# alibaba/unified-audio

Hardware: NVIDIA H100
Metric: hcodec2_encode_rvq_decode_samples_per_s (higher is better)
Workload: dtype f16x3/f16 tensor-core, f32 accumulate

## Files before the change

### unified_audio_b200/csrc/common.cuh

```cuda
#pragma once
#include <cuda.h>
#include <cuda_fp16.h>
#include <cuda_runtime.h>
#include <stdint.h>

namespace qb {

void set_error(const char* fmt, ...);
#define QB_CHECK_CUDA(expr)                                                              \
  do {                                                                                   \
    cudaError_t _e = (expr);                                                             \
    if (_e != cudaSuccess) {                                                             \
      qb::set_error("%s:%d CUDA error %s: %s", __FILE__, __LINE__, #expr, cudaGetErrorString(_e)); \
      return -2;                                                                         \
    }                                                                                    \
  } while (0)
#define QB_REQUIRE(cond, ...)                                                            \
  do {                                                                                   \
    if (!(cond)) {                                                                       \
      qb::set_error(__VA_ARGS__);                                                        \
      return -1;                                                                         \
    }                                                                                    \
  } while (0)

static inline int64_t ceil_div(int64_t a, int64_t b) { return (a + b - 1) / b; }

__device__ __forceinline__ float gelu_erf(float x) { return 0.5f * x * (1.0f + erff(x * 0.70710678118654752440f)); }
__device__ __forceinline__ float gelu_fast(float x) {
  const float z = fabsf(x) * 0.70710678118654752440f;
  float t;
  asm("rcp.approx.ftz.f32 %0, %1;" : "=f"(t) : "f"(fmaf(0.3275911f, z, 1.0f)));
  float p = fmaf(1.061405429f, t, -1.453152027f);
  p = fmaf(p, t, 1.421413741f);
  p = fmaf(p, t, -0.284496736f);
  p = fmaf(p, t, 0.254829592f);
  p *= t;
  float e;
  asm("ex2.approx.ftz.f32 %0, %1;" : "=f"(e) : "f"(-1.4426950408889634f * z * z));
  const float erf_abs = fmaf(-p, e, 1.0f);
  const float half_x = 0.5f * x;
  return fmaf(fabsf(half_x), erf_abs, half_x);
}
__device__ __forceinline__ float sigmoid_f(float x) { return 1.0f / (1.0f + __expf(-x)); }
__device__ __forceinline__ float sigmoid_acc(float x) { return 1.0f / (1.0f + expf(-x)); }
#ifndef LM_ATT_U_DEFAULT
#define LM_ATT_U_DEFAULT 8
#endif
__device__ __forceinline__ float silu_f(float x) { return x / (1.0f + expf(-x)); }
__device__ __forceinline__ float elu_f(float x) { return x > 0.f ? x : expm1f(x); }

__device__ __forceinline__ __half f2h_sat(float x) {
  unsigned short h;
  asm("cvt.rn.satfinite.f16.f32 %0, %1;" : "=h"(h) : "f"(x));
  return __ushort_as_half(h);
}
__device__ __forceinline__ void split_f16(float x, __half& hi, __half& lo) {
  hi = f2h_sat(x);
  lo = __float2half_rn(x - __half2float(hi));
}

__device__ __forceinline__ float warp_sum(float v) {
#pragma unroll
  for (int o = 16; o > 0; o >>= 1) v += __shfl_xor_sync(0xffffffffu, v, o);
  return v;
}
__device__ __forceinline__ float warp_max(float v) {
#pragma unroll
  for (int o = 16; o > 0; o >>= 1) v = fmaxf(v, __shfl_xor_sync(0xffffffffu, v, o));
  return v;
}

__device__ __forceinline__ uint32_t smem_u32(const void* p) { return (uint32_t)__cvta_generic_to_shared(p); }

__device__ __forceinline__ bool elect_one() {
  uint32_t pred;
  asm volatile(
      "{\n\t.reg .pred P;\n\t elect.sync _|P, 0xffffffff;\n\t selp.u32 %0, 1, 0, P;\n\t}\n"
      : "=r"(pred));
  return pred != 0;
}

__device__ __forceinline__ void mbar_init(uint64_t* bar, uint32_t count) {
  asm volatile("mbarrier.init.shared::cta.b64 [%0], %1;" ::"r"(smem_u32(bar)), "r"(count));
}
__device__ __forceinline__ void fence_mbar_init() { asm volatile("fence.mbarrier_init.release.cluster;" ::: "memory"); }
__device__ __forceinline__ void fence_proxy_async() { asm volatile("fence.proxy.async.shared::cta;" ::: "memory"); }
__device__ __forceinline__ void mbar_arrive_expect_tx(uint64_t* bar, uint32_t bytes) {
  asm volatile("mbarrier.arrive.expect_tx.shared::cta.b64 _, [%0], %1;" ::"r"(smem_u32(bar)), "r"(bytes) : "memory");
}
__device__ __forceinline__ void mbar_arrive(uint64_t* bar) {
  asm volatile("mbarrier.arrive.shared::cta.b64 _, [%0];" ::"r"(smem_u32(bar)) : "memory");
}
__device__ __forceinline__ bool mbar_try_wait(uint64_t* bar, uint32_t parity) {
  uint32_t ok;
  asm volatile(
      "{\n\t.reg .pred P;\n\t"
      "mbarrier.try_wait.parity.shared::cta.b64 P, [%1], %2;\n\t"
      "selp.u32 %0, 1, 0, P;\n\t}\n"
      : "=r"(ok)
      : "r"(smem_u32(bar)), "r"(parity)
      : "memory");
  return ok != 0;
}
__device__ __forceinline__ void mbar_wait(uint64_t* bar, uint32_t parity) {
  uint32_t spins = 0;
  while (!mbar_try_wait(bar, parity)) {
    if (++spins > (1u << 26)) { asm volatile("trap;"); }
  }
}

__device__ __forceinline__ void mbar_wait_parked(uint64_t* bar, uint32_t parity) {
  uint32_t spins = 0;
  for (;;) {
    uint32_t ok;
    asm volatile(
        "{\n\t.reg .pred P;\n\t"
        "mbarrier.try_wait.parity.shared::cta.b64 P, [%1], %2, %3;\n\t"
        "selp.u32 %0, 1, 0, P;\n\t}\n"
        : "=r"(ok)
        : "r"(smem_u32(bar)), "r"(parity), "r"(200000u)
        : "memory");
    if (ok) return;
    if (++spins > (1u << 22)) { asm volatile("trap;"); }
  }
}

template <int N>
__device__ __forceinline__ void setmaxnreg_inc() { asm volatile("setmaxnreg.inc.sync.aligned.u32 %0;" ::"n"(N)); }
template <int N>
__device__ __forceinline__ void setmaxnreg_dec() { asm volatile("setmaxnreg.dec.sync.aligned.u32 %0;" ::"n"(N)); }

__device__ __forceinline__ void prefetch_tmap(const void* tmap) {
  asm volatile("prefetch.tensormap [%0];" ::"l"(tmap) : "memory");
}
__device__ __forceinline__ void tma_load_2d(void* smem_dst, const void* tmap, uint64_t* bar, int x, int y) {
  asm volatile(
      "cp.async.bulk.tensor.2d.shared::cluster.global.mbarrier::complete_tx::bytes [%0], [%1, {%3, %4}], [%2];"
      ::"r"(smem_u32(smem_dst)), "l"(tmap), "r"(smem_u32(bar)), "r"(x), "r"(y)
      : "memory");
}
__device__ __forceinline__ void tma_load_3d(void* smem_dst, const void* tmap, uint64_t* bar, int x, int y, int z) {
  asm volatile(
      "cp.async.bulk.tensor.3d.shared::cluster.global.mbarrier::complete_tx::bytes [%0], [%1, {%3, %4, %5}], [%2];"
      ::"r"(smem_u32(smem_dst)), "l"(tmap), "r"(smem_u32(bar)), "r"(x), "r"(y), "r"(z)
      : "memory");
}
__device__ __forceinline__ void tma_store_3d(const void* tmap, const void* smem_src, int x, int y, int z) {
  asm volatile("cp.async.bulk.tensor.3d.global.shared::cta.bulk_group [%0, {%2, %3, %4}], [%1];"
               ::"l"(tmap), "r"(smem_u32(smem_src)), "r"(x), "r"(y), "r"(z)
               : "memory");
}
__device__ __forceinline__ void bulk_commit() { asm volatile("cp.async.bulk.commit_group;" ::: "memory"); }
template <int N>
__device__ __forceinline__ void bulk_wait_read() { asm volatile("cp.async.bulk.wait_group.read %0;" ::"n"(N) : "memory"); }
template <int N>
__device__ __forceinline__ void bulk_wait() { asm volatile("cp.async.bulk.wait_group %0;" ::"n"(N) : "memory"); }
__device__ __forceinline__ void st_shared_f32x2(uint32_t addr, float x, float y) {
  asm volatile("st.shared.v2.f32 [%0], {%1, %2};" ::"r"(addr), "f"(x), "f"(y));
}
__device__ __forceinline__ float2 ld_shared_f32x2(uint32_t addr) {
  float2 v;
  asm volatile("ld.shared.v2.f32 {%0, %1}, [%2];" : "=f"(v.x), "=f"(v.y) : "r"(addr));
  return v;
}
__device__ __forceinline__ void st_shared_b32(uint32_t addr, uint32_t v) {
  asm volatile("st.shared.b32 [%0], %1;" ::"r"(addr), "r"(v));
}
__device__ __forceinline__ void named_bar_sync(int id, int count) {
  asm volatile("bar.sync %0, %1;" ::"r"(id), "r"(count) : "memory");
}

}
```

### unified_audio_b200/csrc/gemm.cu

```cuda
#include <cstdarg>
#include <cstdio>
#include <cstdlib>
#include <cstring>
#include <atomic>

#include "common.cuh"
#include "quark_b200.h"
#include "wgmma.cuh"

namespace qb {

static thread_local char g_err[1024] = "";
std::atomic<long long> g_launches{0};
void set_error(const char* fmt, ...) {
  va_list ap;
  va_start(ap, fmt);
  vsnprintf(g_err, sizeof(g_err), fmt, ap);
  va_end(ap);
}

constexpr int QB_MAX_DEVICES = 64;
static int current_device() {
  int dev = 0;
  cudaGetDevice(&dev);
  return dev >= 0 && dev < QB_MAX_DEVICES ? dev : 0;
}

#ifndef QB_PARK
#define QB_PARK 1
#endif

enum EpiKind : int { EPI_GENERIC = 0, EPI_HI = 1, EPI_F32 = 2 };

struct RowMapD {
  void* ptr;
  long long ld, rpb, off;
};
struct GemmParams {
  int tiles_per_batch, num_n_tiles, num_tiles, num_kb;
  int taps, stride, cblocks, C, dil;
  int Cld;
  int m_per_batch, N;
  const float* bias;
  const float* gamma;
  const float* act_p;
  const float* act2_p;
  RowMapD res, o32, ohi, olo;
  int act, act2;
  int epi;
  const __half *a_hi, *a_lo, *w_hi, *w_lo;
  long long a_rpb;
  int a_batch;
};

__device__ __forceinline__ float snake_f(float v, float a) {
  const float t = a * v;
  float sn;
  if (fabsf(t) < 64.f) {
    const float k = rintf(t * 0.15915494309189535f);
    const float r = fmaf(k, -6.2831854820251465f, t);
    sn = __sinf(fmaf(k, 1.7484555e-7f, r));
  } else {
    sn = sinf(t);
  }
  float rc;
  asm("rcp.approx.ftz.f32 %0, %1;" : "=f"(rc) : "f"(a + 1e-9f));
  return fmaf(rc, sn * sn, v);
}
__device__ __forceinline__ float apply_act(int act, float v) {
  if (act == QB_ACT_GELU) return gelu_fast(v);
  if (act == QB_ACT_ELU) return elu_f(v);
  if (act == QB_ACT_TANH) return tanhf(v);
  if (act == QB_ACT_RELU) return v < 0.f ? 0.f : v;
  return v;
}

__device__ __forceinline__ void epi_finish_scalar(const GemmParams& p, int b, int m, int n, float v) {
  if (p.gamma) v *= __ldg(p.gamma + n);
  if (p.res.ptr) v += ((const float*)p.res.ptr)[((long long)b * p.res.rpb + p.res.off + m) * p.res.ld + n];
  if (p.o32.ptr) ((float*)p.o32.ptr)[((long long)b * p.o32.rpb + p.o32.off + m) * p.o32.ld + n] = v;
  if (p.ohi.ptr) {
    float u = p.act2 == QB_ACT_ELU ? elu_f(v) : (p.act2 == QB_ACT_SNAKE ? snake_f(v, __ldg(p.act2_p + n)) : v);
    __half h, l;
    split_f16(u, h, l);
    long long o = ((long long)b * p.ohi.rpb + p.ohi.off + m) * p.ohi.ld + n;
    ((__half*)p.ohi.ptr)[o] = h;
    if (p.olo.ptr) ((__half*)p.olo.ptr)[o] = l;
  }
}

__device__ __forceinline__ uint8_t* align1024(uint8_t* p) {
  return (uint8_t*)(((uintptr_t)p + 1023) & ~(uintptr_t)1023);
}

__device__ __forceinline__ void epilogue_pair(const GemmParams& p, int b, int m, int n, float v0, float v1) {
  if (m >= p.m_per_batch || n >= p.N) return;
  const bool has1 = n + 1 < p.N;
  if (p.bias) {
    v0 += __ldg(p.bias + n);
    if (has1) v1 += __ldg(p.bias + n + 1);
  }
  if (p.act == QB_ACT_SWIGLU) {
    epi_finish_scalar(p, b, m, n >> 1, silu_f(v0) * v1);
    return;
  }
  if (has1 && p.act2 == QB_ACT_NONE && (p.act == QB_ACT_NONE || p.act == QB_ACT_GELU)) {
    if (p.ohi.ptr && !p.olo.ptr && !p.o32.ptr && !p.res.ptr && !p.gamma && (p.ohi.ld & 1) == 0 &&
        (reinterpret_cast<uintptr_t>(p.ohi.ptr) & 3) == 0) {
      if (p.act == QB_ACT_GELU) { v0 = gelu_fast(v0); v1 = gelu_fast(v1); }
      const __half2 hmax = __float2half2_rn(65504.f), hmin = __float2half2_rn(-65504.f);
      *reinterpret_cast<__half2*>((__half*)p.ohi.ptr + ((long long)b * p.ohi.rpb + p.ohi.off + m) * p.ohi.ld + n) =
          __hmax2_nan(__hmin2_nan(__floats2half2_rn(v0, v1), hmax), hmin);
      return;
    }
    if (p.o32.ptr && !p.ohi.ptr && p.act == QB_ACT_NONE && (p.o32.ld & 1) == 0 && (reinterpret_cast<uintptr_t>(p.o32.ptr) & 7) == 0 &&
        (!p.res.ptr || ((p.res.ld & 1) == 0 && (reinterpret_cast<uintptr_t>(p.res.ptr) & 7) == 0)) &&
        (!p.gamma || (reinterpret_cast<uintptr_t>(p.gamma) & 7) == 0)) {
      if (p.gamma) {
        const float2 g = __ldg(reinterpret_cast<const float2*>(p.gamma + n));
        v0 *= g.x; v1 *= g.y;
      }
      if (p.res.ptr) {
        const float2 r = *reinterpret_cast<const float2*>((const float*)p.res.ptr + ((long long)b * p.res.rpb + p.res.off + m) * p.res.ld + n);
        v0 += r.x; v1 += r.y;
      }
      *reinterpret_cast<float2*>((float*)p.o32.ptr + ((long long)b * p.o32.rpb + p.o32.off + m) * p.o32.ld + n) = make_float2(v0, v1);
      return;
    }
  }
  if (p.act == QB_ACT_SNAKE) {
    v0 = snake_f(v0, __ldg(p.act_p + n));
    if (has1) v1 = snake_f(v1, __ldg(p.act_p + n + 1));
  } else if (p.act != QB_ACT_NONE) {
    v0 = apply_act(p.act, v0);
    v1 = apply_act(p.act, v1);
  }
  epi_finish_scalar(p, b, m, n, v0);
  if (has1) epi_finish_scalar(p, b, m, n + 1, v1);
}

constexpr int GEMM_BM = 128, GEMM_BK = 64;
constexpr int GEMM_THREADS = 3 * 128;
constexpr int GEMM_PRODUCER_REGS = 40, GEMM_CONSUMER_REGS = 232;

constexpr int EPI_BUFS = 2;
constexpr uint32_t EPI_SUB_BYTES = 64 * 128;

template <int BN>
__device__ __forceinline__ void load_tile_cols(const GemmParams& p, int n0, int ct, float (&v)[2 * BN / 256]) {
#pragma unroll
  for (int i = 0; i < 2 * BN / 256; ++i) {
    const int k = ct + 256 * i, n = n0 + k % BN;
    const float* src = k < BN ? p.bias : p.gamma;
    v[i] = src && n < p.N ? __ldg(src + n) : 0.f;
  }
}

struct EpiCtx {
  uint8_t* buf;
  uint64_t* rfull;
  uint32_t cols;
  int cw, b, row0, n0;
};

template <int BN>
__device__ __forceinline__ void epilogue_hi(const GemmParams& p, const CUtensorMap* tmO, const EpiCtx& e, const float (&acc)[BN / 2]) {
  constexpr int NSUB = BN / 64;
  const __half2 hmax = __float2half2_rn(65504.f), hmin = __float2half2_rn(-65504.f);
  const bool gelu = p.act == QB_ACT_GELU, leader = (threadIdx.x & 127) == 0;
  const int lane = threadIdx.x & 31;
  const uint32_t th = smem_u32(e.buf) + (((threadIdx.x >> 5) & 3) * 16 + (lane >> 2)) * 128 + 4 * (lane & 3), sw = (lane >> 2) << 4;
#pragma unroll
  for (int s = 0; s < NSUB; ++s) {
    uint8_t* buf = e.buf + (s % EPI_BUFS) * EPI_SUB_BYTES;
    if (s == 0) {
      if (leader) bulk_wait_read<0>();
      named_bar_sync(2 + e.cw, 128);
    } else if (s >= EPI_BUFS) {
      if (leader) bulk_wait_read<EPI_BUFS - 1>();
      named_bar_sync(2 + e.cw, 128);
    }
#pragma unroll
    for (int jj = 0; jj < 8; ++jj) {
      const int j = 8 * s + jj;
      const float2 bb = p.bias ? ld_shared_f32x2(e.cols + 4 * (8 * j + 2 * (lane & 3))) : make_float2(0.f, 0.f);
#pragma unroll
      for (int h = 0; h < 2; ++h) {
        float v0 = acc[4 * j + 2 * h], v1 = acc[4 * j + 2 * h + 1];
        if (p.bias) { v0 += bb.x; v1 += bb.y; }
        if (gelu) { v0 = gelu_fast(v0); v1 = gelu_fast(v1); }
        const __half2 o = __hmax2_nan(__hmin2_nan(__floats2half2_rn(v0, v1), hmax), hmin);
        st_shared_b32(th + (s % EPI_BUFS) * EPI_SUB_BYTES + h * 1024 + ((16 * jj) ^ sw), *reinterpret_cast<const uint32_t*>(&o));
      }
    }
    fence_proxy_async();
    named_bar_sync(2 + e.cw, 128);
    if (leader) {
      tma_store_3d(tmO, buf, e.n0 + 64 * s, e.row0, e.b);
      bulk_commit();
    }
  }
}

template <int BN>
__device__ __forceinline__ void epilogue_f32(const GemmParams& p, const CUtensorMap* tmO, const CUtensorMap* tmR, const EpiCtx& e,
                                             const float (&acc)[BN / 2]) {
  constexpr int NSUB = BN / 32;
  static_assert(NSUB % (2 * EPI_BUFS) == 0, "each residual barrier completes an even number of phases per tile");
  const bool res = p.res.ptr != nullptr, leader = (threadIdx.x & 127) == 0;
  const int lane = threadIdx.x & 31;
  const uint32_t th = smem_u32(e.buf) + (((threadIdx.x >> 5) & 3) * 16 + (lane >> 2)) * 128 + 8 * (lane & 1),
                 sw = (((lane >> 1) & 1) ^ (lane >> 2)) << 4;
#pragma unroll
  for (int s = 0; s < NSUB; ++s) {
    const int u = s % EPI_BUFS;
    uint8_t* buf = e.buf + u * EPI_SUB_BYTES;
    if (res) {
      mbar_wait(&e.rfull[u], (s / EPI_BUFS) & 1);
    } else if (s == 0) {
      if (leader) bulk_wait_read<0>();
      named_bar_sync(2 + e.cw, 128);
    } else if (s >= EPI_BUFS) {
      if (leader) bulk_wait_read<EPI_BUFS - 1>();
      named_bar_sync(2 + e.cw, 128);
    }
#pragma unroll
    for (int jj = 0; jj < 4; ++jj) {
      const int j = 4 * s + jj;
      const uint32_t col = e.cols + 4 * (8 * j + 2 * (lane & 3));
      const float2 bb = p.bias ? ld_shared_f32x2(col) : make_float2(0.f, 0.f);
      const float2 g = p.gamma ? ld_shared_f32x2(col + 4 * BN) : make_float2(1.f, 1.f);
#pragma unroll
      for (int h = 0; h < 2; ++h) {
        const uint32_t el = th + u * EPI_SUB_BYTES + h * 1024 + ((32 * jj) ^ sw);
        float v0 = acc[4 * j + 2 * h], v1 = acc[4 * j + 2 * h + 1];
        if (p.bias) { v0 += bb.x; v1 += bb.y; }
        if (p.gamma) { v0 *= g.x; v1 *= g.y; }
        if (res) {
          const float2 rv = ld_shared_f32x2(el);
          v0 += rv.x; v1 += rv.y;
        }
        st_shared_f32x2(el, v0, v1);
      }
    }
    fence_proxy_async();
    named_bar_sync(2 + e.cw, 128);
    if (leader) {
      tma_store_3d(tmO, buf, e.n0 + 32 * s, e.row0, e.b);
      bulk_commit();
      if (res && s + EPI_BUFS < NSUB) {
        bulk_wait_read<0>();
        mbar_arrive_expect_tx(&e.rfull[u], EPI_SUB_BYTES);
        tma_load_3d(buf, tmR, &e.rfull[u], e.n0 + 32 * (s + EPI_BUFS), e.row0, e.b);
      }
    }
  }
}

template <int NTERMS, int BN, int STAGES>
__global__ void __launch_bounds__(GEMM_THREADS, 1)
gemm_tc_kernel(const __grid_constant__ CUtensorMap tmA_hi, const __grid_constant__ CUtensorMap tmA_lo,
               const __grid_constant__ CUtensorMap tmW_hi, const __grid_constant__ CUtensorMap tmW_lo,
               const __grid_constant__ CUtensorMap tmOut, const __grid_constant__ CUtensorMap tmRes,
               const GemmParams p) {
  constexpr int BM = GEMM_BM, BK = GEMM_BK;
  constexpr int NPL = (NTERMS == 1) ? 1 : 2;
  constexpr uint32_t A_BYTES = BM * BK * 2, W_BYTES = BN * BK * 2;
  constexpr uint32_t STAGE_BYTES = NPL * (A_BYTES + W_BYTES);
  constexpr int CONSUMER_WARPS = 8;

  extern __shared__ __align__(128) uint8_t smem_raw[];
  uint8_t* smem = align1024(smem_raw);
  uint8_t* epi_smem = smem + STAGES * STAGE_BYTES;
  float* tile_cols = (float*)(epi_smem + 2 * EPI_BUFS * EPI_SUB_BYTES);
  uint64_t* full = (uint64_t*)(tile_cols + 2 * BN);
  uint64_t* empty = full + STAGES;
  uint64_t* rfull = empty + STAGES;

  const int warp = threadIdx.x >> 5, lane = threadIdx.x & 31, wg = warp >> 2;
  const bool tma_epi = p.epi != EPI_GENERIC;
  if (threadIdx.x == 0) {
    for (int s = 0; s < STAGES; ++s) { mbar_init(&full[s], 1); mbar_init(&empty[s], CONSUMER_WARPS); }
    for (int s = 0; s < 2 * EPI_BUFS; ++s) mbar_init(&rfull[s], 1);
    fence_mbar_init();
  }
  if (threadIdx.x == 32) {
    prefetch_tmap(&tmA_hi); prefetch_tmap(&tmW_hi);
    if (NPL == 2) { prefetch_tmap(&tmA_lo); prefetch_tmap(&tmW_lo); }
    if (tma_epi) { prefetch_tmap(&tmOut); if (p.res.ptr) prefetch_tmap(&tmRes); }
  }
  __syncthreads();

  if (wg == 0) {
    setmaxnreg_dec<GEMM_PRODUCER_REGS>();
    if (threadIdx.x == 0) {
      uint32_t stage = 0, phase = 0;
      for (int tile = blockIdx.x; tile < p.num_tiles; tile += gridDim.x) {
        const int n_tile = tile % p.num_n_tiles, m_tile = tile / p.num_n_tiles;
        const int b = m_tile / p.tiles_per_batch, m0 = (m_tile % p.tiles_per_batch) * BM, n0 = n_tile * BN;
        for (int kb = 0; kb < p.num_kb; ++kb) {
          const int tap = kb / p.cblocks, cb = kb - tap * p.cblocks;
          if (QB_PARK) mbar_wait_parked(&empty[stage], phase ^ 1); else mbar_wait(&empty[stage], phase ^ 1);
          mbar_arrive_expect_tx(&full[stage], STAGE_BYTES);
          uint8_t* s = smem + stage * STAGE_BYTES;
          const int tt = tap * p.dil;
          const int ax = (tt % p.stride) * p.Cld + cb * BK, ay = m0 + tt / p.stride, wx = tap * p.C + cb * BK;
          tma_load_3d(s, &tmA_hi, &full[stage], ax, ay, b);
          if (NPL == 2) tma_load_3d(s + A_BYTES, &tmA_lo, &full[stage], ax, ay, b);
          tma_load_2d(s + NPL * A_BYTES, &tmW_hi, &full[stage], wx, n0);
          if (NPL == 2) tma_load_2d(s + NPL * A_BYTES + W_BYTES, &tmW_lo, &full[stage], wx, n0);
          if (++stage == STAGES) { stage = 0; phase ^= 1; }
        }
      }
    }
  } else {
    setmaxnreg_inc<GEMM_CONSUMER_REGS>();
    const int cw = wg - 1, wq = warp & 3;
    const bool leader = (threadIdx.x & 127) == 0, epi_res = p.epi == EPI_F32 && p.res.ptr;
    const bool epi_cols = tma_epi && (p.bias || p.gamma);
    uint32_t stage = 0, phase = 0;
    float acc[BN / 2];
    for (int tile = blockIdx.x; tile < p.num_tiles; tile += gridDim.x) {
      const int n_tile = tile % p.num_n_tiles, m_tile = tile / p.num_n_tiles;
      const int b = m_tile / p.tiles_per_batch, m0 = (m_tile % p.tiles_per_batch) * BM, n0 = n_tile * BN;
      float cols[2 * BN / 256];
      if (epi_cols) load_tile_cols<BN>(p, n0, threadIdx.x - 128, cols);
      uint32_t prev_stage = 0;
      for (int kb = 0; kb < p.num_kb; ++kb) {
        mbar_wait(&full[stage], phase);
        const uint32_t sa = smem_u32(smem + stage * STAGE_BYTES) + cw * (A_BYTES / 2);
        const uint32_t sw = smem_u32(smem + stage * STAGE_BYTES) + NPL * A_BYTES;
        wgmma_fence();
#pragma unroll
        for (int k = 0; k < BK / 16; ++k) {
          const uint64_t a_hi = make_wgmma_desc_sw128(sa + k * 32), w_hi = make_wgmma_desc_sw128(sw + k * 32);
          Wgmma<BN>::ss(acc, a_hi, w_hi, (kb | k) != 0 ? 1u : 0u);
          if (NTERMS == 3) {
            Wgmma<BN>::ss(acc, make_wgmma_desc_sw128(sa + A_BYTES + k * 32), w_hi, 1u);
            Wgmma<BN>::ss(acc, a_hi, make_wgmma_desc_sw128(sw + W_BYTES + k * 32), 1u);
          }
        }
        wgmma_commit();
        if (kb == 0 && epi_res && leader) {
          bulk_wait_read<0>();
#pragma unroll
          for (int u = 0; u < EPI_BUFS; ++u) {
            uint64_t* bar = rfull + cw * EPI_BUFS + u;
            mbar_arrive_expect_tx(bar, EPI_SUB_BYTES);
            tma_load_3d(epi_smem + (cw * EPI_BUFS + u) * EPI_SUB_BYTES, &tmRes, bar, n0 + 32 * u, m0 + cw * 64, b);
          }
        }
        wgmma_wait<1>();
        if (kb > 0 && lane == 0) mbar_arrive(&empty[prev_stage]);
        prev_stage = stage;
        if (++stage == STAGES) { stage = 0; phase ^= 1; }
      }
      wgmma_wait<0>();
      wgmma_fence_regs(acc);
      if (lane == 0) mbar_arrive(&empty[prev_stage]);
      if (epi_cols) {
        named_bar_sync(1, 256);
#pragma unroll
        for (int i = 0; i < 2 * BN / 256; ++i) tile_cols[threadIdx.x - 128 + 256 * i] = cols[i];
        named_bar_sync(1, 256);
      }
      const EpiCtx ec{epi_smem + cw * EPI_BUFS * EPI_SUB_BYTES, rfull + cw * EPI_BUFS, smem_u32(tile_cols), cw, b, m0 + cw * 64, n0};
      if (p.epi == EPI_HI) {
        epilogue_hi<BN>(p, &tmOut, ec, acc);
      } else if (p.epi == EPI_F32) {
        epilogue_f32<BN>(p, &tmOut, &tmRes, ec, acc);
      } else {
        const int r = m0 + cw * 64 + wq * 16 + (lane >> 2), c = n0 + 2 * (lane & 3);
#pragma unroll
        for (int j = 0; j < BN / 8; ++j) {
          epilogue_pair(p, b, r, c + 8 * j, acc[4 * j], acc[4 * j + 1]);
          epilogue_pair(p, b, r + 8, c + 8 * j, acc[4 * j + 2], acc[4 * j + 3]);
        }
      }
    }
    if (tma_epi && leader) bulk_wait<0>();
  }
}

__global__ void gemm_simt_kernel(const GemmParams p) {
  const int N_out = p.act == QB_ACT_SWIGLU ? p.N / 2 : p.N;
  long long gid = (long long)blockIdx.x * blockDim.x + threadIdx.x;
  long long total = (long long)p.a_batch * p.m_per_batch * N_out;
  if (gid >= total) return;
  const int n = (int)(gid % N_out);
  const long long bm = gid / N_out;
  const int m = (int)(bm % p.m_per_batch), b = (int)(bm / p.m_per_batch);
  const long long K = (long long)p.taps * p.C;
  auto dot = [&](int col) {
    float acc = 0.f;
    for (int t = 0; t < p.taps; ++t) {
      long long row = (long long)m * p.stride + (long long)t * p.dil;
      if (row >= p.a_rpb) continue;
      const __half* ah = p.a_hi + ((long long)b * p.a_rpb + row) * p.Cld;
      const __half* al = p.a_lo ? p.a_lo + ((long long)b * p.a_rpb + row) * p.Cld : nullptr;
      const __half* wh = p.w_hi + (long long)col * K + (long long)t * p.C;
      const __half* wl = p.w_lo ? p.w_lo + (long long)col * K + (long long)t * p.C : nullptr;
      for (int c = 0; c < p.C; ++c) {
        float a = __half2float(ah[c]), w = __half2float(wh[c]);
        acc = fmaf(a, w, acc);
        if (al && wl) {
          acc = fmaf(__half2float(al[c]), w, acc);
          acc = fmaf(a, __half2float(wl[c]), acc);
        }
      }
    }
    return acc;
  };
  float v;
  if (p.act == QB_ACT_SWIGLU) {
    float g = dot(2 * n), u = dot(2 * n + 1);
    if (p.bias) { g += p.bias[2 * n]; u += p.bias[2 * n + 1]; }
    v = silu_f(g) * u;
  } else {
    v = dot(n);
    if (p.bias) v += p.bias[n];
    v = p.act == QB_ACT_SNAKE ? snake_f(v, p.act_p[n]) : apply_act(p.act, v);
  }
  epi_finish_scalar(p, b, m, n, v);
}

typedef CUresult (*EncodeTiledFn)(CUtensorMap*, CUtensorMapDataType, cuuint32_t, void*, const cuuint64_t*,
                                  const cuuint64_t*, const cuuint32_t*, const cuuint32_t*, CUtensorMapInterleave,
                                  CUtensorMapSwizzle, CUtensorMapL2promotion, CUtensorMapFloatOOBfill);
static EncodeTiledFn get_encode() {
  static EncodeTiledFn fn = nullptr;
  if (!fn) {
    void* p = nullptr;
    cudaDriverEntryPointQueryResult q;
    if (cudaGetDriverEntryPoint("cuTensorMapEncodeTiled", &p, cudaEnableDefault, &q) == cudaSuccess &&
        q == cudaDriverEntryPointSuccess)
      fn = (EncodeTiledFn)p;
  }
  return fn;
}

static int make_map(CUtensorMap* m, const void* base, int rank, const cuuint64_t* dims, const cuuint64_t* strides_bytes,
                    const cuuint32_t* box, CUtensorMapDataType dtype = CU_TENSOR_MAP_DATA_TYPE_FLOAT16) {
  EncodeTiledFn enc = get_encode();
  QB_REQUIRE(enc != nullptr, "cuTensorMapEncodeTiled not available (no CUDA driver?)");
  cuuint32_t es[3] = {1, 1, 1};
  CUresult r = enc(m, dtype, rank, const_cast<void*>(base), dims, strides_bytes, box, es,
                   CU_TENSOR_MAP_INTERLEAVE_NONE, CU_TENSOR_MAP_SWIZZLE_128B, CU_TENSOR_MAP_L2_PROMOTION_L2_256B,
                   CU_TENSOR_MAP_FLOAT_OOB_FILL_NONE);
  QB_REQUIRE(r == CUDA_SUCCESS, "cuTensorMapEncodeTiled failed: %d (rank %d dims %llu %llu %llu)", (int)r, rank,
             (unsigned long long)dims[0], (unsigned long long)dims[1], (unsigned long long)(rank > 2 ? dims[2] : 0));
  return 0;
}

static RowMapD to_rm(const qb_rowmap& r) { return RowMapD{r.ptr, (long long)r.ld, (long long)r.rows_per_batch, (long long)r.row_off}; }

static bool aligned(const void* ptr, uintptr_t bytes) { return (reinterpret_cast<uintptr_t>(ptr) & (bytes - 1)) == 0; }

static bool tma_rows(const RowMapD& r, long long esize, const GemmParams& p) {
  return r.ld >= p.N && (r.ld * esize) % 16 == 0 && (p.N * esize) % 16 == 0 && aligned(r.ptr, 16) &&
         (p.a_batch == 1 || r.rpb >= r.off + p.m_per_batch);
}

static int classify_epilogue(const GemmParams& p) {
  if (p.act2 != QB_ACT_NONE) return EPI_GENERIC;
  if (p.ohi.ptr && !p.olo.ptr && !p.o32.ptr && !p.res.ptr && !p.gamma && (p.act == QB_ACT_NONE || p.act == QB_ACT_GELU) &&
      tma_rows(p.ohi, 2, p))
    return EPI_HI;
  if (p.o32.ptr && !p.ohi.ptr && p.act == QB_ACT_NONE && tma_rows(p.o32, 4, p) && (!p.res.ptr || tma_rows(p.res, 4, p)))
    return EPI_F32;
  return EPI_GENERIC;
}

static int make_rows_map(CUtensorMap* m, const RowMapD& r, bool f32, const GemmParams& p) {
  const cuuint64_t es = f32 ? 4 : 2, ld = (cuuint64_t)r.ld;
  const cuuint64_t rows = p.a_batch > 1 ? (cuuint64_t)r.rpb : (cuuint64_t)p.m_per_batch;
  cuuint64_t dims[3] = {(cuuint64_t)p.N, (cuuint64_t)p.m_per_batch, (cuuint64_t)p.a_batch};
  cuuint64_t str[2] = {ld * es, rows * ld * es};
  cuuint32_t box[3] = {(cuuint32_t)(128 / es), 64, 1};
  return make_map(m, (const char*)r.ptr + r.off * ld * es, 3, dims, str, box,
                  f32 ? CU_TENSOR_MAP_DATA_TYPE_FLOAT32 : CU_TENSOR_MAP_DATA_TYPE_FLOAT16);
}

static int fill_params(const qb_gemm_desc* d, GemmParams* p, int BN) {
  QB_REQUIRE(d && d->a_hi && d->w_hi, "gemm: null operand");
  QB_REQUIRE((d->a_lo == nullptr) == (d->w_lo == nullptr), "gemm: a_lo and w_lo must both be given or both be NULL");
  QB_REQUIRE(d->taps >= 1 && d->stride >= 1, "gemm: bad taps/stride");
  QB_REQUIRE(d->a_ld % 64 == 0 && d->a_ld > 0, "gemm: a_ld (%lld) must be a positive multiple of 64", (long long)d->a_ld);
  QB_REQUIRE(d->a_rows_per_batch % d->stride == 0, "gemm: a_rows_per_batch must be a multiple of stride");
  QB_REQUIRE(d->a_batch >= 1 && d->m_per_batch >= 1 && d->n >= 1, "gemm: empty problem");
  QB_REQUIRE(d->act != QB_ACT_SWIGLU || d->n % 2 == 0, "gemm: SWIGLU needs even n");
  QB_REQUIRE(!d->out_lo.ptr || d->out_hi.ptr, "gemm: out_lo without out_hi");
  QB_REQUIRE(d->act != QB_ACT_SNAKE || d->act_param, "gemm: QB_ACT_SNAKE needs act_param (alpha[n])");
  QB_REQUIRE(d->act2 != QB_ACT_SNAKE || (d->act2_param && (reinterpret_cast<uintptr_t>(d->act2_param) & 7) == 0),
             "gemm: act2 = QB_ACT_SNAKE needs an 8-byte aligned act2_param (alpha[n])");
  memset(p, 0, sizeof(*p));
  p->tiles_per_batch = (int)ceil_div(d->m_per_batch, 128);
  p->num_n_tiles = (int)ceil_div(d->n, BN);
  p->num_tiles = (int)(d->a_batch * p->tiles_per_batch * p->num_n_tiles);
  const int64_t ck = d->a_cols > 0 ? d->a_cols : d->a_ld;
  QB_REQUIRE(ck % 64 == 0 && ck <= d->a_ld, "gemm: a_cols (%lld) must be a multiple of 64 and <= a_ld", (long long)ck);
  p->taps = d->taps; p->stride = d->stride; p->C = (int)ck; p->Cld = (int)d->a_ld; p->cblocks = (int)(ck / 64);
  p->dil = d->dilation > 0 ? d->dilation : 1;
  p->num_kb = p->taps * p->cblocks;
  p->m_per_batch = (int)d->m_per_batch; p->N = (int)d->n;
  p->bias = d->bias; p->gamma = d->gamma; p->act_p = d->act_param; p->act2_p = d->act2_param;
  p->res = to_rm(d->residual); p->o32 = to_rm(d->out_f32); p->ohi = to_rm(d->out_hi); p->olo = to_rm(d->out_lo);
  if (p->olo.ptr) { p->olo.ld = p->ohi.ld; p->olo.rpb = p->ohi.rpb; p->olo.off = p->ohi.off; }
  p->act = d->act; p->act2 = d->act2;
  p->a_hi = (const __half*)d->a_hi; p->a_lo = (const __half*)d->a_lo;
  p->w_hi = (const __half*)d->w_hi; p->w_lo = (const __half*)d->w_lo;
  p->a_rpb = d->a_rows_per_batch; p->a_batch = (int)d->a_batch;
  p->epi = classify_epilogue(*p);
  return 0;
}

template <int NTERMS, int BN, int STAGES>
static int launch_tc(const qb_gemm_desc* d, cudaStream_t st, int num_sms) {
  GemmParams p;
  if (int e = fill_params(d, &p, BN)) return e;
  CUtensorMap mA_hi, mA_lo, mW_hi, mW_lo;
  const cuuint64_t C = (cuuint64_t)d->a_ld, s = (cuuint64_t)d->stride;
  cuuint64_t adims[3] = {s * C, (cuuint64_t)d->a_rows_per_batch / s, (cuuint64_t)d->a_batch};
  cuuint64_t astr[2] = {s * C * 2, (cuuint64_t)d->a_rows_per_batch * C * 2};
  cuuint32_t abox[3] = {64, 128, 1};
  const cuuint64_t Ck = (cuuint64_t)(d->a_cols > 0 ? d->a_cols : d->a_ld);
  cuuint64_t wdims[2] = {(cuuint64_t)d->taps * Ck, (cuuint64_t)d->n};
  cuuint64_t wstr[1] = {(cuuint64_t)d->taps * Ck * 2};
  cuuint32_t wbox[2] = {64, (cuuint32_t)BN};
  if (int e = make_map(&mA_hi, d->a_hi, 3, adims, astr, abox)) return e;
  if (int e = make_map(&mW_hi, d->w_hi, 2, wdims, wstr, wbox)) return e;
  if (NTERMS == 3) {
    if (int e = make_map(&mA_lo, d->a_lo, 3, adims, astr, abox)) return e;
    if (int e = make_map(&mW_lo, d->w_lo, 2, wdims, wstr, wbox)) return e;
  } else {
    mA_lo = mA_hi; mW_lo = mW_hi;
  }
  CUtensorMap mOut = mA_hi, mRes = mA_hi;
  if (p.epi == EPI_HI) {
    if (int e = make_rows_map(&mOut, p.ohi, false, p)) return e;
  } else if (p.epi == EPI_F32) {
    if (int e = make_rows_map(&mOut, p.o32, true, p)) return e;
    if (p.res.ptr)
      if (int e = make_rows_map(&mRes, p.res, true, p)) return e;
  }
  constexpr int NPL = NTERMS == 1 ? 1 : 2;
  constexpr size_t smem = (size_t)STAGES * NPL * (GEMM_BM * 64 * 2 + BN * 64 * 2) + 2 * EPI_BUFS * EPI_SUB_BYTES + 2 * BN * 4 +
                          (2 * STAGES + 2 * EPI_BUFS) * 8 + 1024 - 128;
  static_assert(smem <= 227 * 1024, "GEMM pipeline and epilogue buffers exceed the 227 KB of shared memory a block may use");
  auto kern = gemm_tc_kernel<NTERMS, BN, STAGES>;
  static bool attr_set[QB_MAX_DEVICES] = {};
  const int dev = current_device();
  if (!attr_set[dev]) {
    QB_CHECK_CUDA(cudaFuncSetAttribute(kern, cudaFuncAttributeMaxDynamicSharedMemorySize, (int)smem));
    attr_set[dev] = true;
  }
  int grid = p.num_tiles < num_sms ? p.num_tiles : num_sms;
  kern<<<grid, GEMM_THREADS, smem, st>>>(mA_hi, mA_lo, mW_hi, mW_lo, mOut, mRes, p);
  g_launches++;
  QB_CHECK_CUDA(cudaGetLastError());
  return 0;
}

static int num_sms_cached() {
  static int n[QB_MAX_DEVICES] = {};
  const int dev = current_device();
  if (!n[dev]) {
    cudaDeviceGetAttribute(&n[dev], cudaDevAttrMultiProcessorCount, dev);
    if (const char* e = getenv("QB_GEMM_SMS")) n[dev] = atoi(e);
  }
  return n[dev];
}

}

using namespace qb;

extern "C" const char* qb_last_error(void) { return g_err; }
extern "C" int qb_version(void) { return 100; }
extern "C" int64_t qb_launch_count(void) { return (int64_t)g_launches.load(); }
extern "C" void qb_launch_count_reset(void) { g_launches = 0; }

extern "C" const char* qb_gemm_kernel_name(int64_t m_per_batch, int64_t n, int32_t split) {
  (void)m_per_batch;
  if (split) return "gemm_tc_kernel<3,128,3>";
  return n > 128 ? "gemm_tc_kernel<1,256,4>" : "gemm_tc_kernel<1,128,6>";
}

extern "C" int qb_gemm(const qb_gemm_desc* d, void* stream) {
  cudaStream_t st = (cudaStream_t)stream;
  QB_REQUIRE(d != nullptr, "gemm: null desc");
  const int sms = num_sms_cached();
  if (d->a_lo != nullptr) return launch_tc<3, 128, 3>(d, st, sms);
  return d->n > 128 ? launch_tc<1, 256, 4>(d, st, sms) : launch_tc<1, 128, 6>(d, st, sms);
}

extern "C" int qb_gemm_simt(const qb_gemm_desc* d, void* stream) {
  GemmParams p;
  if (int e = fill_params(d, &p, 128)) return e;
  const long long n_out = d->act == QB_ACT_SWIGLU ? d->n / 2 : d->n;
  const long long total = d->a_batch * d->m_per_batch * n_out;
  gemm_simt_kernel<<<(unsigned)ceil_div(total, 256), 256, 0, (cudaStream_t)stream>>>(p);
  g_launches++;
  QB_CHECK_CUDA(cudaGetLastError());
  return 0;
}
```

Baseline: 125.2 million.

## Route split-f16 hi/lo, ELU and SwiGLU outputs through the TMA-store epilogue

Broadens the TMA-store epilogues so more GEMM variants avoid the generic per-thread global-store epilogue. The hi epilogue now handles ELU and SwiGLU activations and writes both hi and lo f16 planes. The f32 epilogue can also emit hi/lo f16 planes with an optional ELU, using 64B-swizzled tensor maps. It costs extra tensor-map parameters, single-buffered epilogue staging when planes are written (less store overlap), and more branches in the epilogue code.

Result: faster. 143.4 million (median of 6 runs) (+14.5%).

```diff
diff --git a/unified_audio_b200/csrc/common.cuh b/unified_audio_b200/csrc/common.cuh
--- a/unified_audio_b200/csrc/common.cuh
+++ b/unified_audio_b200/csrc/common.cuh
@@ -166,6 +166,9 @@
 __device__ __forceinline__ void st_shared_b32(uint32_t addr, uint32_t v) {
   asm volatile("st.shared.b32 [%0], %1;" ::"r"(addr), "r"(v));
 }
+__device__ __forceinline__ void st_shared_b16(uint32_t addr, __half v) {
+  asm volatile("st.shared.b16 [%0], %1;" ::"r"(addr), "h"(__half_as_ushort(v)));
+}
 __device__ __forceinline__ void named_bar_sync(int id, int count) {
   asm volatile("bar.sync %0, %1;" ::"r"(id), "r"(count) : "memory");
 }
diff --git a/unified_audio_b200/csrc/gemm.cu b/unified_audio_b200/csrc/gemm.cu
--- a/unified_audio_b200/csrc/gemm.cu
+++ b/unified_audio_b200/csrc/gemm.cu
@@ -163,17 +163,21 @@
   int cw, b, row0, n0;
 };
 
-template <int BN>
-__device__ __forceinline__ void epilogue_hi(const GemmParams& p, const CUtensorMap* tmO, const EpiCtx& e, const float (&acc)[BN / 2]) {
-  constexpr int NSUB = BN / 64;
+template <int BN, bool SWIGLU>
+__device__ __forceinline__ void epilogue_hi(const GemmParams& p, const CUtensorMap* tmHi, const CUtensorMap* tmLo, const EpiCtx& e,
+                                                const float (&acc)[BN / 2]) {
+  constexpr int NSUB = SWIGLU ? BN / 128 : BN / 64, JS = SWIGLU ? 16 : 8;
   const __half2 hmax = __float2half2_rn(65504.f), hmin = __float2half2_rn(-65504.f);
-  const bool gelu = p.act == QB_ACT_GELU, leader = (threadIdx.x & 127) == 0;
+  const int act = p.act;
+  const bool lo = BN == 128 && p.olo.ptr != nullptr, leader = (threadIdx.x & 127) == 0;
+  const bool rn_sat = BN == 256 || (!lo && (act == QB_ACT_NONE || act == QB_ACT_GELU));
   const int lane = threadIdx.x & 31;
-  const uint32_t th = smem_u32(e.buf) + (((threadIdx.x >> 5) & 3) * 16 + (lane >> 2)) * 128 + 4 * (lane & 3), sw = (lane >> 2) << 4;
+  const uint32_t th = smem_u32(e.buf) + (((threadIdx.x >> 5) & 3) * 16 + (lane >> 2)) * 128 + (SWIGLU ? 2 : 4) * (lane & 3),
+                 sw = (lane >> 2) << 4;
 #pragma unroll
   for (int s = 0; s < NSUB; ++s) {
-    uint8_t* buf = e.buf + (s % EPI_BUFS) * EPI_SUB_BYTES;
-    if (s == 0) {
+    const uint32_t bh = (lo ? 0 : s % EPI_BUFS) * EPI_SUB_BYTES, bl = EPI_SUB_BYTES;
+    if (s == 0 || lo) {
       if (leader) bulk_wait_read<0>();
       named_bar_sync(2 + e.cw, 128);
     } else if (s >= EPI_BUFS) {
@@ -181,43 +185,66 @@
       named_bar_sync(2 + e.cw, 128);
     }
 #pragma unroll
-    for (int jj = 0; jj < 8; ++jj) {
-      const int j = 8 * s + jj;
+    for (int jj = 0; jj < JS; ++jj) {
+      const int j = JS * s + jj;
       const float2 bb = p.bias ? ld_shared_f32x2(e.cols + 4 * (8 * j + 2 * (lane & 3))) : make_float2(0.f, 0.f);
 #pragma unroll
       for (int h = 0; h < 2; ++h) {
         float v0 = acc[4 * j + 2 * h], v1 = acc[4 * j + 2 * h + 1];
         if (p.bias) { v0 += bb.x; v1 += bb.y; }
-        if (gelu) { v0 = gelu_fast(v0); v1 = gelu_fast(v1); }
-        const __half2 o = __hmax2_nan(__hmin2_nan(__floats2half2_rn(v0, v1), hmax), hmin);
-        st_shared_b32(th + (s % EPI_BUFS) * EPI_SUB_BYTES + h * 1024 + ((16 * jj) ^ sw), *reinterpret_cast<const uint32_t*>(&o));
+        if (SWIGLU) {
+          const uint32_t el = th + h * 1024 + ((16 * (jj >> 1)) ^ sw) + 8 * (jj & 1);
+          __half hv, lv;
+          split_f16(silu_f(v0) * v1, hv, lv);
+          st_shared_b16(el + bh, hv);
+          if (lo) st_shared_b16(el + bl, lv);
+        } else {
+          const uint32_t el = th + h * 1024 + ((16 * jj) ^ sw);
+          if (act == QB_ACT_GELU) { v0 = gelu_fast(v0); v1 = gelu_fast(v1); }
+          else if (BN == 128 && act == QB_ACT_ELU) { v0 = elu_f(v0); v1 = elu_f(v1); }
+          if (rn_sat) {
+            const __half2 o = __hmax2_nan(__hmin2_nan(__floats2half2_rn(v0, v1), hmax), hmin);
+            st_shared_b32(el + bh, *reinterpret_cast<const uint32_t*>(&o));
+          } else {
+            __half2 hv, lv;
+            split_f16(v0, hv.x, lv.x);
+            split_f16(v1, hv.y, lv.y);
+            st_shared_b32(el + bh, *reinterpret_cast<const uint32_t*>(&hv));
+            if (lo) st_shared_b32(el + bl, *reinterpret_cast<const uint32_t*>(&lv));
+          }
+        }
       }
     }
     fence_proxy_async();
     named_bar_sync(2 + e.cw, 128);
     if (leader) {
-      tma_store_3d(tmO, buf, e.n0 + 64 * s, e.row0, e.b);
+      const int x = (SWIGLU ? e.n0 / 2 : e.n0) + 64 * s;
+      tma_store_3d(tmHi, e.buf + bh, x, e.row0, e.b);
+      if (lo) tma_store_3d(tmLo, e.buf + bl, x, e.row0, e.b);
       bulk_commit();
     }
   }
 }
 
 template <int BN>
-__device__ __forceinline__ void epilogue_f32(const GemmParams& p, const CUtensorMap* tmO, const CUtensorMap* tmR, const EpiCtx& e,
-                                             const float (&acc)[BN / 2]) {
+__device__ __forceinline__ void epilogue_f32(const GemmParams& p, const CUtensorMap* tmO, const CUtensorMap* tmR, const CUtensorMap* tmHi,
+                                             const CUtensorMap* tmLo, const EpiCtx& e, const float (&acc)[BN / 2]) {
   constexpr int NSUB = BN / 32;
+  constexpr uint32_t LO_OFF = EPI_SUB_BYTES / 2;
   static_assert(NSUB % (2 * EPI_BUFS) == 0, "each residual barrier completes an even number of phases per tile");
-  const bool res = p.res.ptr != nullptr, leader = (threadIdx.x & 127) == 0;
-  const int lane = threadIdx.x & 31;
-  const uint32_t th = smem_u32(e.buf) + (((threadIdx.x >> 5) & 3) * 16 + (lane >> 2)) * 128 + 8 * (lane & 1),
-                 sw = (((lane >> 1) & 1) ^ (lane >> 2)) << 4;
+  const bool res = p.res.ptr != nullptr, planes = BN == 128 && p.ohi.ptr != nullptr, lo = p.olo.ptr != nullptr;
+  const bool elu = p.act2 == QB_ACT_ELU;
+  const bool leader = (threadIdx.x & 127) == 0;
+  const int lane = threadIdx.x & 31, row = ((threadIdx.x >> 5) & 3) * 16 + (lane >> 2);
+  const uint32_t th = smem_u32(e.buf) + row * 128 + 8 * (lane & 1), sw = (((lane >> 1) & 1) ^ (lane >> 2)) << 4;
+  const uint32_t tp = smem_u32(e.buf + EPI_SUB_BYTES) + row * 64 + 4 * (lane & 3), swp = ((lane >> 3) & 3) << 4;
 #pragma unroll
   for (int s = 0; s < NSUB; ++s) {
-    const int u = s % EPI_BUFS;
+    const int u = planes ? 0 : s % EPI_BUFS;
     uint8_t* buf = e.buf + u * EPI_SUB_BYTES;
     if (res) {
-      mbar_wait(&e.rfull[u], (s / EPI_BUFS) & 1);
-    } else if (s == 0) {
+      mbar_wait(&e.rfull[u], (planes ? s : s / EPI_BUFS) & 1);
+    } else if (s == 0 || planes) {
       if (leader) bulk_wait_read<0>();
       named_bar_sync(2 + e.cw, 128);
     } else if (s >= EPI_BUFS) {
@@ -241,17 +268,31 @@
           v0 += rv.x; v1 += rv.y;
         }
         st_shared_f32x2(el, v0, v1);
+        if (planes) {
+          if (elu) { v0 = elu_f(v0); v1 = elu_f(v1); }
+          const uint32_t ep = tp + h * 512 + ((16 * jj) ^ swp);
+          __half2 hv, lv;
+          split_f16(v0, hv.x, lv.x);
+          split_f16(v1, hv.y, lv.y);
+          st_shared_b32(ep, *reinterpret_cast<const uint32_t*>(&hv));
+          if (lo) st_shared_b32(ep + LO_OFF, *reinterpret_cast<const uint32_t*>(&lv));
+        }
       }
     }
     fence_proxy_async();
     named_bar_sync(2 + e.cw, 128);
     if (leader) {
       tma_store_3d(tmO, buf, e.n0 + 32 * s, e.row0, e.b);
+      if (planes) {
+        tma_store_3d(tmHi, e.buf + EPI_SUB_BYTES, e.n0 + 32 * s, e.row0, e.b);
+        if (lo) tma_store_3d(tmLo, e.buf + EPI_SUB_BYTES + LO_OFF, e.n0 + 32 * s, e.row0, e.b);
+      }
       bulk_commit();
-      if (res && s + EPI_BUFS < NSUB) {
+      const int next = s + (planes ? 1 : EPI_BUFS);
+      if (res && next < NSUB) {
         bulk_wait_read<0>();
         mbar_arrive_expect_tx(&e.rfull[u], EPI_SUB_BYTES);
-        tma_load_3d(buf, tmR, &e.rfull[u], e.n0 + 32 * (s + EPI_BUFS), e.row0, e.b);
+        tma_load_3d(buf, tmR, &e.rfull[u], e.n0 + 32 * next, e.row0, e.b);
       }
     }
   }
@@ -262,7 +303,7 @@
 gemm_tc_kernel(const __grid_constant__ CUtensorMap tmA_hi, const __grid_constant__ CUtensorMap tmA_lo,
                const __grid_constant__ CUtensorMap tmW_hi, const __grid_constant__ CUtensorMap tmW_lo,
                const __grid_constant__ CUtensorMap tmOut, const __grid_constant__ CUtensorMap tmRes,
-               const GemmParams p) {
+               const __grid_constant__ CUtensorMap tmHi, const __grid_constant__ CUtensorMap tmLo, const GemmParams p) {
   constexpr int BM = GEMM_BM, BK = GEMM_BK;
   constexpr int NPL = (NTERMS == 1) ? 1 : 2;
   constexpr uint32_t A_BYTES = BM * BK * 2, W_BYTES = BN * BK * 2;
@@ -287,7 +328,8 @@
   if (threadIdx.x == 32) {
     prefetch_tmap(&tmA_hi); prefetch_tmap(&tmW_hi);
     if (NPL == 2) { prefetch_tmap(&tmA_lo); prefetch_tmap(&tmW_lo); }
-    if (tma_epi) { prefetch_tmap(&tmOut); if (p.res.ptr) prefetch_tmap(&tmRes); }
+    if (p.epi == EPI_F32) { prefetch_tmap(&tmOut); if (p.res.ptr) prefetch_tmap(&tmRes); }
+    if (tma_epi && p.ohi.ptr) { prefetch_tmap(&tmHi); if (p.olo.ptr) prefetch_tmap(&tmLo); }
   }
   __syncthreads();
 
@@ -317,6 +359,7 @@
     setmaxnreg_inc<GEMM_CONSUMER_REGS>();
     const int cw = wg - 1, wq = warp & 3;
     const bool leader = (threadIdx.x & 127) == 0, epi_res = p.epi == EPI_F32 && p.res.ptr;
+    const int res_bufs = BN == 128 && p.ohi.ptr ? 1 : EPI_BUFS;
     const bool epi_cols = tma_epi && (p.bias || p.gamma);
     uint32_t stage = 0, phase = 0;
     float acc[BN / 2];
@@ -343,8 +386,7 @@
         wgmma_commit();
         if (kb == 0 && epi_res && leader) {
           bulk_wait_read<0>();
-#pragma unroll
-          for (int u = 0; u < EPI_BUFS; ++u) {
+          for (int u = 0; u < res_bufs; ++u) {
             uint64_t* bar = rfull + cw * EPI_BUFS + u;
             mbar_arrive_expect_tx(bar, EPI_SUB_BYTES);
             tma_load_3d(epi_smem + (cw * EPI_BUFS + u) * EPI_SUB_BYTES, &tmRes, bar, n0 + 32 * u, m0 + cw * 64, b);
@@ -366,9 +408,14 @@
       }
       const EpiCtx ec{epi_smem + cw * EPI_BUFS * EPI_SUB_BYTES, rfull + cw * EPI_BUFS, smem_u32(tile_cols), cw, b, m0 + cw * 64, n0};
       if (p.epi == EPI_HI) {
-        epilogue_hi<BN>(p, &tmOut, ec, acc);
+        if constexpr (BN == 128) {
+          if (p.act == QB_ACT_SWIGLU) epilogue_hi<BN, true>(p, &tmHi, &tmLo, ec, acc);
+          else epilogue_hi<BN, false>(p, &tmHi, &tmLo, ec, acc);
+        } else {
+          epilogue_hi<BN, false>(p, &tmHi, &tmLo, ec, acc);
+        }
       } else if (p.epi == EPI_F32) {
-        epilogue_f32<BN>(p, &tmOut, &tmRes, ec, acc);
+        epilogue_f32<BN>(p, &tmOut, &tmRes, &tmHi, &tmLo, ec, acc);
       } else {
         const int r = m0 + cw * 64 + wq * 16 + (lane >> 2), c = n0 + 2 * (lane & 3);
 #pragma unroll
@@ -440,12 +487,13 @@
 }
 
 static int make_map(CUtensorMap* m, const void* base, int rank, const cuuint64_t* dims, const cuuint64_t* strides_bytes,
-                    const cuuint32_t* box, CUtensorMapDataType dtype = CU_TENSOR_MAP_DATA_TYPE_FLOAT16) {
+                    const cuuint32_t* box, CUtensorMapDataType dtype = CU_TENSOR_MAP_DATA_TYPE_FLOAT16,
+                    CUtensorMapSwizzle swizzle = CU_TENSOR_MAP_SWIZZLE_128B) {
   EncodeTiledFn enc = get_encode();
   QB_REQUIRE(enc != nullptr, "cuTensorMapEncodeTiled not available (no CUDA driver?)");
   cuuint32_t es[3] = {1, 1, 1};
   CUresult r = enc(m, dtype, rank, const_cast<void*>(base), dims, strides_bytes, box, es,
-                   CU_TENSOR_MAP_INTERLEAVE_NONE, CU_TENSOR_MAP_SWIZZLE_128B, CU_TENSOR_MAP_L2_PROMOTION_L2_256B,
+                   CU_TENSOR_MAP_INTERLEAVE_NONE, swizzle, CU_TENSOR_MAP_L2_PROMOTION_L2_256B,
                    CU_TENSOR_MAP_FLOAT_OOB_FILL_NONE);
   QB_REQUIRE(r == CUDA_SUCCESS, "cuTensorMapEncodeTiled failed: %d (rank %d dims %llu %llu %llu)", (int)r, rank,
              (unsigned long long)dims[0], (unsigned long long)dims[1], (unsigned long long)(rank > 2 ? dims[2] : 0));
@@ -456,29 +504,35 @@
 
 static bool aligned(const void* ptr, uintptr_t bytes) { return (reinterpret_cast<uintptr_t>(ptr) & (bytes - 1)) == 0; }
 
+static int out_cols(const GemmParams& p) { return p.act == QB_ACT_SWIGLU ? p.N / 2 : p.N; }
+
 static bool tma_rows(const RowMapD& r, long long esize, const GemmParams& p) {
-  return r.ld >= p.N && (r.ld * esize) % 16 == 0 && (p.N * esize) % 16 == 0 && aligned(r.ptr, 16) &&
+  return r.ld >= out_cols(p) && (r.ld * esize) % 16 == 0 && (out_cols(p) * esize) % 16 == 0 && aligned(r.ptr, 16) &&
          (p.a_batch == 1 || r.rpb >= r.off + p.m_per_batch);
 }
 
-static int classify_epilogue(const GemmParams& p) {
-  if (p.act2 != QB_ACT_NONE) return EPI_GENERIC;
-  if (p.ohi.ptr && !p.olo.ptr && !p.o32.ptr && !p.res.ptr && !p.gamma && (p.act == QB_ACT_NONE || p.act == QB_ACT_GELU) &&
-      tma_rows(p.ohi, 2, p))
+static int classify_epilogue(const GemmParams& p, int BN) {
+  const bool wide = BN == 256;
+  const bool planes_ok = !p.ohi.ptr || (tma_rows(p.ohi, 2, p) && (!p.olo.ptr || tma_rows(p.olo, 2, p)));
+  if (p.ohi.ptr && !p.o32.ptr && !p.res.ptr && !p.gamma && p.act2 == QB_ACT_NONE && planes_ok &&
+      (wide ? !p.olo.ptr && (p.act == QB_ACT_NONE || p.act == QB_ACT_GELU)
+            : p.act == QB_ACT_NONE || p.act == QB_ACT_GELU || p.act == QB_ACT_ELU || p.act == QB_ACT_SWIGLU))
     return EPI_HI;
-  if (p.o32.ptr && !p.ohi.ptr && p.act == QB_ACT_NONE && tma_rows(p.o32, 4, p) && (!p.res.ptr || tma_rows(p.res, 4, p)))
+  if (p.o32.ptr && p.act == QB_ACT_NONE && (wide ? !p.ohi.ptr : p.act2 == QB_ACT_NONE || p.act2 == QB_ACT_ELU) && planes_ok &&
+      tma_rows(p.o32, 4, p) && (!p.res.ptr || tma_rows(p.res, 4, p)))
     return EPI_F32;
   return EPI_GENERIC;
 }
 
-static int make_rows_map(CUtensorMap* m, const RowMapD& r, bool f32, const GemmParams& p) {
+static int make_rows_map(CUtensorMap* m, const RowMapD& r, bool f32, int box_bytes, const GemmParams& p) {
   const cuuint64_t es = f32 ? 4 : 2, ld = (cuuint64_t)r.ld;
   const cuuint64_t rows = p.a_batch > 1 ? (cuuint64_t)r.rpb : (cuuint64_t)p.m_per_batch;
-  cuuint64_t dims[3] = {(cuuint64_t)p.N, (cuuint64_t)p.m_per_batch, (cuuint64_t)p.a_batch};
+  cuuint64_t dims[3] = {(cuuint64_t)out_cols(p), (cuuint64_t)p.m_per_batch, (cuuint64_t)p.a_batch};
   cuuint64_t str[2] = {ld * es, rows * ld * es};
-  cuuint32_t box[3] = {(cuuint32_t)(128 / es), 64, 1};
+  cuuint32_t box[3] = {(cuuint32_t)(box_bytes / es), 64, 1};
   return make_map(m, (const char*)r.ptr + r.off * ld * es, 3, dims, str, box,
-                  f32 ? CU_TENSOR_MAP_DATA_TYPE_FLOAT32 : CU_TENSOR_MAP_DATA_TYPE_FLOAT16);
+                  f32 ? CU_TENSOR_MAP_DATA_TYPE_FLOAT32 : CU_TENSOR_MAP_DATA_TYPE_FLOAT16,
+                  box_bytes == 128 ? CU_TENSOR_MAP_SWIZZLE_128B : CU_TENSOR_MAP_SWIZZLE_64B);
 }
 
 static int fill_params(const qb_gemm_desc* d, GemmParams* p, int BN) {
@@ -510,7 +564,7 @@
   p->a_hi = (const __half*)d->a_hi; p->a_lo = (const __half*)d->a_lo;
   p->w_hi = (const __half*)d->w_hi; p->w_lo = (const __half*)d->w_lo;
   p->a_rpb = d->a_rows_per_batch; p->a_batch = (int)d->a_batch;
-  p->epi = classify_epilogue(*p);
+  p->epi = classify_epilogue(*p, BN);
   return 0;
 }
 
@@ -535,13 +589,17 @@
   } else {
     mA_lo = mA_hi; mW_lo = mW_hi;
   }
-  CUtensorMap mOut = mA_hi, mRes = mA_hi;
-  if (p.epi == EPI_HI) {
-    if (int e = make_rows_map(&mOut, p.ohi, false, p)) return e;
-  } else if (p.epi == EPI_F32) {
-    if (int e = make_rows_map(&mOut, p.o32, true, p)) return e;
+  CUtensorMap mOut = mA_hi, mRes = mA_hi, mHi = mA_hi, mLo = mA_hi;
+  if (p.epi == EPI_F32) {
+    if (int e = make_rows_map(&mOut, p.o32, true, 128, p)) return e;
     if (p.res.ptr)
-      if (int e = make_rows_map(&mRes, p.res, true, p)) return e;
+      if (int e = make_rows_map(&mRes, p.res, true, 128, p)) return e;
+  }
+  if (p.epi != EPI_GENERIC && p.ohi.ptr) {
+    const int box_bytes = p.epi == EPI_HI ? 128 : 64;
+    if (int e = make_rows_map(&mHi, p.ohi, false, box_bytes, p)) return e;
+    if (p.olo.ptr)
+      if (int e = make_rows_map(&mLo, p.olo, false, box_bytes, p)) return e;
   }
   constexpr int NPL = NTERMS == 1 ? 1 : 2;
   constexpr size_t smem = (size_t)STAGES * NPL * (GEMM_BM * 64 * 2 + BN * 64 * 2) + 2 * EPI_BUFS * EPI_SUB_BYTES + 2 * BN * 4 +
@@ -555,7 +613,7 @@
     attr_set[dev] = true;
   }
   int grid = p.num_tiles < num_sms ? p.num_tiles : num_sms;
-  kern<<<grid, GEMM_THREADS, smem, st>>>(mA_hi, mA_lo, mW_hi, mW_lo, mOut, mRes, p);
+  kern<<<grid, GEMM_THREADS, smem, st>>>(mA_hi, mA_lo, mW_hi, mW_lo, mOut, mRes, mHi, mLo, p);
   g_launches++;
   QB_CHECK_CUDA(cudaGetLastError());
   return 0;
```
